# bayesiains/nflows

Hardware: NVIDIA H100
Metric: Flow.log_prob samples/sec, 10-layer RQ-NSF D=784 (higher is better)
Workload: dtype f32

## Files before the change

### nflows_b200/csrc/fused_spline.cuh

```cuda
#pragma once
#include "rq_spline.cuh"
#include "tc_common.cuh"

namespace nfk {
namespace tc {

constexpr int AFFINE_NB = 0;

constexpr int mog_nb(int mp) { return -mp / 8; }

template <int NB, bool TAILS>
struct FusedCfg {
    static constexpr bool AFFINE = NB == AFFINE_NB;
    static constexpr bool MOG = NB < 0;
    static constexpr int M = AFFINE ? 2 : (MOG ? -8 * NB : (TAILS ? 3 * NB - 1 : 3 * NB + 1));
    static constexpr int MP = AFFINE ? 2 : (M + 7) / 8 * 8;
    static constexpr int FPT = BN / (2 * MP);
    static constexpr int TF = 2 * FPT;
    static constexpr int TILE = TF * MP;
    static constexpr int LD = (TILE + 31) / 32 * 32;
    static_assert(FPT >= 1, "unsupported bin count for the fused kernels");
    static_assert(!(AFFINE && TAILS), "the affine epilogue has no tails");
    static_assert(!MOG || (!TAILS && MP <= 64), "mixture epilogue: no tails, at most 64 rows per feature");
};

struct MogOut {
    const float* u;
    const float* e;
    int64_t ldn;
    float eps;
    int C;
    int sample;
};

struct SplineOut {
    const float* bias;
    const float* x;
    float* y;
    __half* y_hi;
    __half* y_lo;
    const int32_t* t_cols;
    int t_col0;
    float out_scale;
    int64_t ldx, ldy, lds;
    int d_t;
    int inverse;
    float inv_acc_scale;
    SplineParams sp;
};

template <int NB, bool TAILS>
__device__ __forceinline__ int stg_chunk(int r, int c) {
    constexpr int C = FusedCfg<NB, TAILS>::FPT * FusedCfg<NB, TAILS>::MP / 4;
    return c ^ ((0x6530 >> (4 * (r & 3))) & 7) ^ ((C % 8 == 0 && c >= C) ? 4 : 0);
}

template <int NB, bool TAILS, int N, int LD = BN>
__device__ __forceinline__ void stage_sums(float* stg, const float (&sum)[N / 2], int wi, int lane) {
    static_assert(N <= LD && LD % 32 == 0, "staged row stride");
#pragma unroll
    for (int j = 0; j < N / 8; ++j)
#pragma unroll
        for (int h = 0; h < 2; ++h) {
            const int r = wi * 16 + (lane >> 2) + 8 * h, c = 2 * j + ((lane & 3) >> 1);
            *reinterpret_cast<float2*>(stg + r * LD + 4 * stg_chunk<NB, TAILS>(r, c) + 2 * (lane & 1)) =
                make_float2(sum[4 * j + 2 * h], sum[4 * j + 2 * h + 1]);
        }
}

template <int NB, bool TAILS>
struct SplineIn {
    float x[FusedCfg<NB, TAILS>::FPT];
    int col[FusedCfg<NB, TAILS>::FPT];
};
template <bool TAILS>
struct SplineIn<AFFINE_NB, TAILS> {};
template <int NB, bool TAILS>
__device__ __forceinline__ SplineIn<NB, TAILS> spline_inputs(const SplineOut& o, int n, int64_t row, bool row_ok, int fh) {
    constexpr int FPT = FusedCfg<NB, TAILS>::FPT, TF = FusedCfg<NB, TAILS>::TF;
    SplineIn<NB, TAILS> in;
    if constexpr (!FusedCfg<NB, TAILS>::AFFINE) {
        const int j0 = n * TF + fh * FPT;
#pragma unroll
        for (int f = 0; f < FPT; ++f) {
            const bool ok = row_ok && (j0 + f < o.d_t) && (!FusedCfg<NB, TAILS>::MOG || o.x != nullptr);
            in.col[f] = !ok ? 0 : (o.t_cols ? __ldg(o.t_cols + j0 + f) : o.t_col0 + j0 + f);
            in.x[f] = ok ? o.x[row * o.ldx + in.col[f]] : 0.0f;
        }
    }
    return in;
}

template <int NB, bool TAILS>
__device__ __forceinline__ void bias_tile_async(float* dst, const SplineOut& o, int n, int t) {
    constexpr int TILE = FusedCfg<NB, TAILS>::TILE, MP = FusedCfg<NB, TAILS>::MP;
    if constexpr (FusedCfg<NB, TAILS>::AFFINE) {
        if (t < TILE / 2) {
            const int e = n * TILE + 2 * t;
            const uint32_t bytes = e < o.d_t * MP ? 8u : 0u;
            asm volatile("cp.async.ca.shared.global [%0], [%1], 8, %2;" ::"r"(smem_u32(dst + 2 * t)), "l"(o.bias + (bytes ? e : 0)),
                         "r"(bytes)
                         : "memory");
        }
    } else if (t < TILE / 4) {
        const int e = n * TILE + 4 * t;
        const uint32_t bytes = e < o.d_t * MP ? 16u : 0u;
        asm volatile("cp.async.cg.shared.global [%0], [%1], 16, %2;" ::"r"(smem_u32(dst + 4 * t)), "l"(o.bias + (bytes ? e : 0)),
                     "r"(bytes)
                     : "memory");
    }
}
__device__ __forceinline__ void cp_async_wait_all() { asm volatile("cp.async.wait_all;" ::: "memory"); }

template <int NB, bool TAILS, int LD, bool BIAS_SMEM>
__device__ __forceinline__ void affine_tile(const SplineOut& o, const float* stg, int r, int n, int64_t row, bool row_ok, int fh,
                                            float& lad_row, const float* bias_tile) {
    using Cfg = FusedCfg<NB, TAILS>;
    constexpr int FPT = Cfg::FPT, TF = Cfg::TF, TILE = Cfg::TILE, C = FPT * 2 / 4;
    const int j0 = n * TF + fh * FPT;
    const int64_t c0 = (int64_t)o.t_col0 + j0;
    const float* b = o.bias + (int64_t)n * TILE + fh * FPT * 2;
    float lad = 0.0f;
    constexpr int G = 8;
#pragma unroll
    for (int g = 0; g < FPT; g += G) {
        float x[G];
#pragma unroll
        for (int f = 0; f < G; ++f) x[f] = (row_ok && j0 + g + f < o.d_t) ? __ldg(o.x + row * o.ldx + c0 + g + f) : 0.0f;
#pragma unroll
        for (int i = g / 2; i < (g + G) / 2; ++i) {
            const float4 s = *reinterpret_cast<const float4*>(stg + r * LD + 4 * stg_chunk<NB, TAILS>(r, fh * C + i));
            const float sv[4] = {s.x, s.y, s.z, s.w};
            float bv[4];
            if constexpr (BIAS_SMEM) {
                const float4 bq = *reinterpret_cast<const float4*>(bias_tile + fh * FPT * 2 + 4 * i);
                bv[0] = bq.x; bv[1] = bq.y; bv[2] = bq.z; bv[3] = bq.w;
            } else {
#pragma unroll
                for (int e = 0; e < 4; ++e) bv[e] = (j0 + 2 * i + e / 2 < o.d_t) ? __ldg(b + 4 * i + e) : 0.0f;
            }
#pragma unroll
            for (int h = 0; h < 2; ++h) {
                const int f = 2 * i + h;
                if (!(row_ok && j0 + f < o.d_t)) continue;
                const float u = fmaf(sv[2 * h], o.inv_acc_scale, bv[2 * h]);
                const float shift = fmaf(sv[2 * h + 1], o.inv_acc_scale, bv[2 * h + 1]);
                const float scale = __fadd_rn(softplus_torch(u, 1.0f, 1.0f), 1e-3f);
                const float xf = x[f - g];
                const float y = o.inverse ? __fdiv_rn(__fsub_rn(xf, shift), scale) : __fadd_rn(__fmul_rn(scale, xf), shift);
                o.y[row * o.ldy + c0 + f] = y;
                lad = __fadd_rn(lad, logf(scale));
            }
        }
    }
    lad_row += o.inverse ? -lad : lad;
}

template <int NB, bool TAILS, int LD>
__device__ __forceinline__ void mog_tile(const SplineOut& o, const MogOut& g, const float* stg, int r, int n, int64_t row, bool row_ok,
                                         int fh, const SplineIn<NB, TAILS>& in, float& lad_row, const float* bias_tile) {
    using Cfg = FusedCfg<NB, TAILS>;
    constexpr int MP = Cfg::MP, FPT = Cfg::FPT, TF = Cfg::TF, C4 = FPT * MP / 4, CMAX = MP / 3;
    constexpr float LOG_2PI = 1.8378770664093453f;
    const int j0 = n * TF + fh * FPT;
    float v[FPT * MP];
#pragma unroll
    for (int i = 0; i < C4; ++i) {
        const float4 s = *reinterpret_cast<const float4*>(stg + r * LD + 4 * stg_chunk<NB, TAILS>(r, fh * C4 + i));
        const float4 bq = *reinterpret_cast<const float4*>(bias_tile + fh * FPT * MP + 4 * i);
        v[4 * i + 0] = fmaf(s.x, o.inv_acc_scale, bq.x);
        v[4 * i + 1] = fmaf(s.y, o.inv_acc_scale, bq.y);
        v[4 * i + 2] = fmaf(s.z, o.inv_acc_scale, bq.z);
        v[4 * i + 3] = fmaf(s.w, o.inv_acc_scale, bq.w);
    }
    float lp = 0.0f;
#pragma unroll
    for (int f = 0; f < FPT; ++f) {
        if (!(row_ok && j0 + f < o.d_t)) continue;
        const float* q = v + f * MP;
        float lmax = -INFINITY;
#pragma unroll
        for (int c = 0; c < CMAX; ++c)
            if (c < g.C) lmax = fmaxf(lmax, q[3 * c]);
        float se = 0.0f;
#pragma unroll
        for (int c = 0; c < CMAX; ++c)
            if (c < g.C) se = __fadd_rn(se, expf(__fsub_rn(q[3 * c], lmax)));
        const int64_t col = (int64_t)o.t_col0 + j0 + f;
        if (!g.sample) {
            const float lse = logf(se), x = in.x[f];
            float t[CMAX];
            float tmax = -INFINITY;
#pragma unroll
            for (int c = 0; c < CMAX; ++c) {
                if (c >= g.C) continue;
                const float sigma = __fadd_rn(softplus_torch(q[3 * c + 2], 1.0f, 1.0f), g.eps);
                const float z = __fdiv_rn(__fsub_rn(x, q[3 * c + 1]), sigma);
                const float quad = __fadd_rn(__fadd_rn(LOG_2PI, __fmul_rn(2.0f, logf(sigma))), __fmul_rn(z, z));
                t[c] = __fsub_rn(__fsub_rn(__fsub_rn(q[3 * c], lmax), lse), __fmul_rn(0.5f, quad));
                tmax = fmaxf(tmax, t[c]);
            }
            float st = 0.0f;
#pragma unroll
            for (int c = 0; c < CMAX; ++c)
                if (c < g.C) st = __fadd_rn(st, expf(__fsub_rn(t[c], tmax)));
            lp = __fadd_rn(lp, __fadd_rn(logf(st), tmax));
        } else {
            const float uu = __ldg(g.u + row * g.ldn + j0 + f), ee = __ldg(g.e + row * g.ldn + j0 + f);
            float cum = 0.0f, mu = 0.0f, us = 0.0f;
            bool found = false;
#pragma unroll
            for (int c = 0; c < CMAX; ++c) {
                if (c >= g.C) continue;
                cum = __fadd_rn(cum, __fdiv_rn(expf(__fsub_rn(q[3 * c], lmax)), se));
                if (!found && (uu < cum || c == g.C - 1)) {
                    found = true;
                    mu = q[3 * c + 1];
                    us = q[3 * c + 2];
                }
            }
            const float sigma = __fadd_rn(softplus_torch(us, 1.0f, 1.0f), g.eps);
            o.y[row * o.ldy + col] = __fadd_rn(mu, __fmul_rn(ee, sigma));
        }
    }
    lad_row += lp;
}

template <int NB, bool TAILS, int LD = BN, bool BIAS_SMEM = false>
__device__ __forceinline__ void spline_tile(const SplineOut& o, const float* stg, int r, int n, int64_t row, bool row_ok, int fh,
                                            const SplineIn<NB, TAILS>& in, float& lad_row, int& flag,
                                            const float* bias_tile = nullptr) {
    using Cfg = FusedCfg<NB, TAILS>;
    if constexpr (Cfg::AFFINE) {
        affine_tile<NB, TAILS, LD, BIAS_SMEM>(o, stg, r, n, row, row_ok, fh, lad_row, bias_tile);
    } else {
        constexpr int MP = Cfg::MP, FPT = Cfg::FPT, TF = Cfg::TF, TILE = Cfg::TILE, C = FPT * MP / 4;
        const int j0 = n * TF + fh * FPT;
        float v[FPT * MP];
        const float* b = o.bias + (int64_t)n * TILE + fh * FPT * MP;
#pragma unroll
        for (int i = 0; i < C; ++i) {
            const float4 s = *reinterpret_cast<const float4*>(stg + r * LD + 4 * stg_chunk<NB, TAILS>(r, fh * C + i));
            const float sv[4] = {s.x, s.y, s.z, s.w};
            if constexpr (BIAS_SMEM) {
                const float4 bq = *reinterpret_cast<const float4*>(bias_tile + fh * FPT * MP + 4 * i);
                const float bv[4] = {bq.x, bq.y, bq.z, bq.w};
#pragma unroll
                for (int e = 0; e < 4; ++e) v[4 * i + e] = fmaf(sv[e], o.inv_acc_scale, bv[e]);
            } else {
#pragma unroll
                for (int e = 0; e < 4; ++e) {
                    const int c = 4 * i + e;
                    v[c] = fmaf(sv[e], o.inv_acc_scale, (j0 + c / MP < o.d_t) ? __ldg(b + c) : 0.0f);
                }
            }
        }
        float yy[FPT], ll[FPT];
        if (o.inverse) rqs_eval_lean<NB, TAILS, true, FPT, MP>(o.sp, in.x, v, yy, ll, flag);
        else rqs_eval_lean<NB, TAILS, false, FPT, MP>(o.sp, in.x, v, yy, ll, flag);
#pragma unroll
        for (int f = 0; f < FPT; ++f) {
            if (!(row_ok && j0 + f < o.d_t)) continue;
            lad_row += ll[f];
            if (o.y_hi) {
                __half hi, lo;
                split_f16(yy[f], o.out_scale, hi, lo, flag);
                o.y_hi[row * o.lds + in.col[f]] = hi;
                o.y_lo[row * o.lds + in.col[f]] = lo;
            } else {
                o.y[row * o.ldy + in.col[f]] = yy[f];
            }
        }
    }
}

}
}
```

### nflows_b200/csrc/nfk_coupling_step_tc.cu

```cuda
#include <stdlib.h>
#include <string.h>

#include <type_traits>

#include "fused_spline.cuh"

namespace nfk {
namespace tc {

constexpr int STEP_MAX_LAYERS = 9;
static_assert(STEP_MAX_LAYERS == NFK_STEP_MAX_LAYERS, "include/nfk.h: NfkStepRowTerms");
constexpr int STEP_MAX_HIDDEN = 256;
constexpr int STEP_DRAIN_TRUNK = 4;
constexpr int STEP_DRAIN_FINAL = 8;
constexpr int STEP_SLAB_BYTES = 2 * A_BYTES;
constexpr int STEP_R_BYTES = (STEP_MAX_HIDDEN / BK) * STEP_SLAB_BYTES;
constexpr int STEP_G0_STAGES = STEP_R_BYTES / STAGE_BYTES;
constexpr int STEP_S_OFF = STEP_R_BYTES;
constexpr int STEP_S_WG_BYTES = 32768;
constexpr int STEP_W_OFF = STEP_S_OFF + 2 * STEP_S_WG_BYTES;
constexpr int STEP_W_STAGES = 2;
constexpr int STEP_W_STAGE_BYTES = 2 * B_BYTES;
constexpr int STEP_BAR_OFF = STEP_W_OFF + STEP_W_STAGES * STEP_W_STAGE_BYTES;
constexpr int STEP_LAD_OFF = STEP_BAR_OFF + 256;
constexpr int STEP_BIAS_OFF = STEP_LAD_OFF + 512;
constexpr int STEP_SMEM_BYTES = STEP_BIAS_OFF + 2 * BN * 4 + 1024 ;
static_assert(64 * BN * 4 <= STEP_S_WG_BYTES && 4 * 2 * 64 * 64 <= STEP_S_WG_BYTES, "S");
static_assert(STEP_SMEM_BYTES <= 232448, "coupling-step kernel shared memory");
static_assert(STEP_MAX_HIDDEN / BK <= STEP_DRAIN_FINAL, "the final layer drains once (mma_final)");

template <int NB, bool TAILS>
struct StepFinal {
    static constexpr int TILE = FusedCfg<NB, TAILS>::TILE, LD = FusedCfg<NB, TAILS>::LD;
    static constexpr int STG_BYTES = 64 * LD * 4;
    static constexpr int RING_OFF = STEP_S_OFF + 2 * STG_BYTES;
    static constexpr int LO_OFF = TILE * ROW_BYTES;
    static constexpr int STAGE_BYTES = 2 * LO_OFF;
    static constexpr int STAGES = (STEP_BAR_OFF - RING_OFF) / STAGE_BYTES;
    static constexpr bool OWN_RING = STAGES > STEP_W_STAGES;
    static_assert(STG_BYTES <= STEP_S_WG_BYTES, "S");
    static_assert(RING_OFF % 512 == 0 && LO_OFF % 512 == 0 && STAGE_BYTES % 512 == 0, "final ring alignment");
    static_assert(!OWN_RING || (STAGES == 4 && RING_OFF >= STEP_S_OFF + STEP_S_WG_BYTES), "final ring");
    static_assert(112 + 2 * 8 * STAGES <= STEP_LAD_OFF - STEP_BAR_OFF, "its mbarriers follow bar_sfree");
};

#ifdef NFK_STEP_CLOCKS
constexpr int CLK_CTAS = 8, CLK_ROUNDS = 3, CLK_TILES = 128, CLK_TILE_STAMPS = 8;
constexpr int CLK_REC = 4 + CLK_TILES * CLK_TILE_STAMPS;
__device__ long long g_step_clocks[CLK_CTAS * CLK_ROUNDS * CLK_REC];
#define NFK_CLK(ptr, i) \
    do {                \
        if (ptr) (ptr)[i] = clock64(); \
    } while (0)
__device__ __forceinline__ long long* step_clock_record(int u, int t) {
    const int round = (u - (int)blockIdx.x) / (int)gridDim.x;
    if (t != 0 || blockIdx.x >= CLK_CTAS || round < 1 || round > CLK_ROUNDS) return nullptr;
    return g_step_clocks + ((int)blockIdx.x * CLK_ROUNDS + round - 1) * CLK_REC;
}
#define NFK_CLK_RECORD(u, t) step_clock_record(u, t)
#define NFK_CLK_TILE(rec, n) ((rec) && (n) < CLK_TILES ? (rec) + 4 + (n) * CLK_TILE_STAMPS : nullptr)
#else
#define NFK_CLK(ptr, i) \
    do {                \
    } while (0)
#define NFK_CLK_RECORD(u, t) ((long long*)nullptr)
#define NFK_CLK_TILE(rec, n) ((long long*)nullptr)
#endif

constexpr int SL_RELU_OUT = 1;
constexpr int SL_ADD_SKIP = 2;
constexpr int SL_SAVE_SKIP = 4;
constexpr int SL_SPLIT_RELU = 8;
constexpr int SL_ACT_SHIFT = 8;
constexpr int SL_ACT_MASK = 15;

__host__ __device__ __forceinline__ int layer_act(int lf) {
    const int a = (lf >> SL_ACT_SHIFT) & SL_ACT_MASK;
    return a ? a : NFK_ACT_RELU;
}

template <int ACT>
__device__ __forceinline__ void act_frag(float (&v)[64]) {
#pragma unroll
    for (int i = 0; i < 64; ++i) v[i] = nfk_act(ACT, v[i]);
}

__device__ __forceinline__ void act_fragment(int act, float (&v)[64]) {
    switch (act) {
        case NFK_ACT_RELU: act_frag<NFK_ACT_RELU>(v); break;
        case NFK_ACT_TANH: act_frag<NFK_ACT_TANH>(v); break;
        case NFK_ACT_ELU: act_frag<NFK_ACT_ELU>(v); break;
        case NFK_ACT_LEAKY_RELU: act_frag<NFK_ACT_LEAKY_RELU>(v); break;
        case NFK_ACT_GELU: act_frag<NFK_ACT_GELU>(v); break;
        case NFK_ACT_SILU: act_frag<NFK_ACT_SILU>(v); break;
    }
}

struct StepParams {
    const float* bias_trunk;
    float* skip_buf;
    int H, K0, num_layers;
    int layer_flags[STEP_MAX_LAYERS];
    float acc_scale[STEP_MAX_LAYERS], inv_acc_scale[STEP_MAX_LAYERS];
    float act_scale;
    __half* h_hi;
    __half* h_lo;
    int64_t ldh;
    SplineOut o;
    float* lad_accum;
    int32_t* flags;
    int64_t n_rows;
    int num_m_tiles, num_n_tiles;
};

struct StepTermParams : StepParams {
    const float* add[STEP_MAX_LAYERS];
    int64_t ld_add[STEP_MAX_LAYERS];
};

struct StepMogParams : StepTermParams {
    MogOut mog;
};

template <int NB, bool TERMS>
using StepParamsOf = typename std::conditional<FusedCfg<NB, false>::MOG, StepMogParams,
                                               typename std::conditional<TERMS, StepTermParams, StepParams>::type>::type;

__device__ __forceinline__ void put_pair(uint8_t* base, int slab_stride, int lo_off, int r, int col, float x0, float x1, float scale,
                                         float& amax) {
    x0 *= scale; x1 *= scale;
    amax = fmaxf(amax, fmaxf(fabsf(x0), fabsf(x1)));
    const __half2 h = __floats2half2_rn(x0, x1);
    const float2 hf = __half22float2(h);
    const __half2 l = __floats2half2_rn(x0 - hf.x, x1 - hf.y);
    const int k = col & 31;
    uint8_t* q = base + (col >> 5) * slab_stride + r * 64 + (((k >> 3) ^ ((r >> 1) & 3)) << 4) + (k & 7) * 2;
    *reinterpret_cast<__half2*>(q) = h;
    *reinterpret_cast<__half2*>(q + lo_off) = l;
}

__device__ __forceinline__ void consumers_sync() { asm volatile("bar.sync 3, 256;" ::: "memory"); }
constexpr int STEP_BAR_TURN = 4;
constexpr int STEP_BAR_LAD = 6;

template <int N, int MH>
__device__ __forceinline__ void mma_final(float (&acc)[MH][N / 2], Ring& r, int num_k, uint32_t a_res, int lane, int turn,
                                          uint32_t lo_off, [[maybe_unused]] long long* clk) {
    int prev = -1;
    for (int j = 0; j < num_k; ++j) {
        mbar_wait(r.full + 8 * r.stage, r.phase);
        if (j == 0) NFK_CLK(clk, 1);
        if (j == num_k - 1) NFK_CLK(clk, 2);
        if (turn >= 0 && j == num_k - 1) {
            __threadfence_block();
            pair_arrive(turn);
        }
        const uint32_t sw = r.base + r.stage * r.stage_bytes;
        const uint64_t w_hi = make_smem_desc(sw), w_lo = make_smem_desc(sw + lo_off);
        wgmma_fence();
#pragma unroll
        for (int m = 0; m < MH; ++m) {
            const uint32_t sa = a_res + (uint32_t)j * STEP_SLAB_BYTES + m * (A_BYTES / 2);
            const uint64_t a_hi = make_smem_desc(sa), a_lo = make_smem_desc(sa + A_BYTES);
#pragma unroll
            for (int kk = 0; kk < BK / 16; ++kk) {
                const uint64_t adv = (uint64_t)(kk * 2);
                wgmma_f16<N>(acc[m], a_lo + adv, w_hi + adv, (j | kk) != 0);
                wgmma_f16<N>(acc[m], a_hi + adv, w_lo + adv, 1);
            }
#pragma unroll
            for (int kk = 0; kk < BK / 16; ++kk) {
                const uint64_t adv = (uint64_t)(kk * 2);
                wgmma_f16<N>(acc[m], a_hi + adv, w_hi + adv, 1);
            }
        }
        wgmma_commit();
        if (prev >= 0) {
            wgmma_wait<1>();
            __syncwarp();
            if (lane == 0) mbar_arrive(r.empty + 8 * prev, MH);
        }
        prev = r.stage;
        r.advance();
    }
    wgmma_wait<0>();
    NFK_CLK(clk, 3);
    __syncwarp();
    if (lane == 0) mbar_arrive(r.empty + 8 * prev, MH);
}

template <int NB, bool TAILS, bool TERMS, bool ACT>
__global__ void __launch_bounds__(THREADS, 1)
rq_coupling_step_kernel(const __grid_constant__ CUtensorMap map_a_hi, const __grid_constant__ CUtensorMap map_a_lo,
                        const __grid_constant__ CUtensorMap map_w0_hi, const __grid_constant__ CUtensorMap map_w0_lo,
                        const __grid_constant__ CUtensorMap map_wt_hi, const __grid_constant__ CUtensorMap map_wt_lo,
                        const __grid_constant__ CUtensorMap map_wf_hi, const __grid_constant__ CUtensorMap map_wf_lo,
                        const StepParamsOf<NB, TERMS> p) {
    using F = StepFinal<NB, TAILS>;
    constexpr int TILE = F::TILE;
    extern __shared__ uint8_t smem_raw[];
    const uint32_t smem_base = (smem_u32(smem_raw) + 1023u) & ~1023u;
    uint8_t* smem_gen = smem_raw + (smem_base - smem_u32(smem_raw));
    const uint32_t bars = smem_base + STEP_BAR_OFF;
    Ring ring0{smem_base, bars, bars + 8 * STEP_G0_STAGES, STEP_G0_STAGES, (uint32_t)STAGE_BYTES};
    Ring ring1{smem_base + STEP_W_OFF, bars + 64, bars + 64 + 8 * STEP_W_STAGES, STEP_W_STAGES, (uint32_t)STEP_W_STAGE_BYTES};
    Ring ring_own{smem_base + F::RING_OFF, bars + 112, bars + 112 + 8 * F::STAGES, F::STAGES, (uint32_t)F::STAGE_BYTES};
    Ring& ringf = F::OWN_RING ? ring_own : ring1;
    constexpr uint32_t lo_f = F::OWN_RING ? F::LO_OFF : B_BYTES;
    const uint32_t bar_rfree = bars + 96;
    const uint32_t bar_sfree = bars + 104;
    const int warp = threadIdx.x >> 5, lane = threadIdx.x & 31;
    const int H = p.H;
    const int num_k0 = (p.K0 + BK - 1) / BK, num_kh = H / BK;
    const int nch = (H + BN - 1) / BN;
    const bool trunk_only = p.h_hi != nullptr;

    if (threadIdx.x == 0) {
        for (int s = 0; s < STEP_G0_STAGES; ++s) { mbar_init(ring0.full + 8 * s, 1); mbar_init(ring0.empty + 8 * s, 8); }
        for (int s = 0; s < STEP_W_STAGES; ++s) { mbar_init(ring1.full + 8 * s, 1); mbar_init(ring1.empty + 8 * s, 8); }
        mbar_init(bar_rfree, 8);
        if constexpr (F::OWN_RING) {
            for (int s = 0; s < F::STAGES; ++s) { mbar_init(ring_own.full + 8 * s, 1); mbar_init(ring_own.empty + 8 * s, 8); }
            mbar_init(bar_sfree, 1);
        }
        asm volatile("fence.mbarrier_init.release.cluster;" ::: "memory");
        prefetch_tmap(&map_a_hi); prefetch_tmap(&map_a_lo); prefetch_tmap(&map_w0_hi); prefetch_tmap(&map_w0_lo);
        prefetch_tmap(&map_wt_hi); prefetch_tmap(&map_wt_lo); prefetch_tmap(&map_wf_hi); prefetch_tmap(&map_wf_lo);
    }
    __syncthreads();

    if (warp < 4) {
        asm volatile("setmaxnreg.dec.sync.aligned.u32 40;" ::: "memory");
        if (warp == 0 && elect_one()) {
            uint32_t rphase = 0, sphase = 0;
            for (int u = blockIdx.x; u < p.num_m_tiles; u += gridDim.x) {
                if (u != (int)blockIdx.x) { mbar_wait(bar_rfree, rphase); rphase ^= 1; }
                for (int c = 0; c < nch; ++c)
                    for (int ks = 0; ks < num_k0; ++ks) produce_slab(ring0, &map_a_hi, &map_a_lo, &map_w0_hi, &map_w0_lo, ks, u * BM, c * BN);
                for (int l = 1; l < p.num_layers; ++l)
                    for (int c = 0; c < nch; ++c)
                        for (int ks = 0; ks < num_kh; ++ks) produce_w_slab(ring1, &map_wt_hi, &map_wt_lo, ks, (l - 1) * H + c * BN);
                if (trunk_only) continue;
                if (F::OWN_RING && p.num_n_tiles > 1) {
                    mbar_wait(bar_sfree, sphase);
                    sphase ^= 1;
                    Ring w = ring1;
                    for (int s = 0; s < STEP_W_STAGES; ++s) {
                        mbar_wait(w.empty + 8 * w.stage, w.phase ^ 1);
                        w.advance();
                    }
                    for (int n = 0; n < p.num_n_tiles; ++n)
                        for (int ks = 0; ks < num_kh; ++ks) produce_w_slab(ring_own, &map_wf_hi, &map_wf_lo, ks, n * TILE, TILE, F::LO_OFF);
                } else {
                    for (int n = 0; n < p.num_n_tiles; ++n)
                        for (int ks = 0; ks < num_kh; ++ks) produce_w_slab(ring1, &map_wf_hi, &map_wf_lo, ks, n * TILE, TILE);
                }
            }
        }
        return;
    }
    asm volatile("setmaxnreg.inc.sync.aligned.u32 232;" ::: "memory");
    const int wg = (warp >> 2) - 1, wi = warp & 3, q = lane & 3;
    const int t = threadIdx.x - 128 * (1 + wg);
    const int r_loc = t >> 1, fh = t & 1;
    uint8_t* R = smem_gen;
    uint8_t* S = smem_gen + STEP_S_OFF + wg * STEP_S_WG_BYTES;
    float* stg = reinterpret_cast<float*>(S);
    float* const bias_wg = reinterpret_cast<float*>(smem_gen + STEP_BIAS_OFF) + wg * BN;
    float* skip = p.skip_buf + (size_t)blockIdx.x * BM * H;
    int flag = 0;
    for (int u = blockIdx.x; u < p.num_m_tiles; u += gridDim.x) {
        const int64_t m0 = (int64_t)u * BM;
        int rt[2];
        rt[0] = wg * 64 + wi * 16 + (lane >> 2);
        rt[1] = rt[0] + 8;
        [[maybe_unused]] long long* const clk = NFK_CLK_RECORD(u, t);
        NFK_CLK(clk, 2 * wg);
        for (int l = 0; l < p.num_layers; ++l) {
            const int lf = p.layer_flags[l];
            [[maybe_unused]] const int act = layer_act(lf);
            const bool to_global = trunk_only && l == p.num_layers - 1;
            const float as = p.acc_scale[l], ias = p.inv_acc_scale[l];
            float amax = 0.0f;
            for (int c = 0; c < nch; ++c) {
                const int cb = c * BN + 2 * q;
                float sum[64];
#pragma unroll
                for (int j = 0; j < 16; ++j) {
                    const int col = cb + 8 * j;
                    [[maybe_unused]] float2 tv[2] = {make_float2(0.0f, 0.0f), make_float2(0.0f, 0.0f)};
                    if constexpr (TERMS) {
                        const float* ta = p.add[l];
                        if (ta != nullptr && col < H) {
#pragma unroll
                            for (int h = 0; h < 2; ++h) {
                                const int64_t row = m0 + rt[h];
                                if (row < p.n_rows) tv[h] = __ldg(reinterpret_cast<const float2*>(ta + row * p.ld_add[l] + col));
                            }
                        }
                    }
#pragma unroll
                    for (int e = 0; e < 2; ++e) {
                        const float b = col < H ? __ldg(p.bias_trunk + l * H + col + e) * as : 0.0f;
#pragma unroll
                        for (int h = 0; h < 2; ++h) {
                            float sk = ((lf & SL_ADD_SKIP) && col < H) ? skip[rt[h] * H + col + e] : 0.0f;
                            if constexpr (TERMS) sk += e ? tv[h].y : tv[h].x;
                            sum[4 * j + 2 * h + e] = fmaf(sk, as, b);
                        }
                    }
                }
                if (l == 0) mma_tile(sum, ring0, num_k0, STEP_DRAIN_TRUNK, wg, lane);
                else mma_tile(sum, ring1, num_kh, STEP_DRAIN_TRUNK, wg, lane, smem_base);
#pragma unroll
                for (int i = 0; i < 64; ++i) {
                    float x = sum[i] * ias;
                    if (!ACT && (lf & SL_RELU_OUT)) x = fmaxf(x, 0.0f);
                    sum[i] = x;
                }
                if (ACT && (lf & SL_RELU_OUT)) act_fragment(act, sum);
                if (lf & SL_SAVE_SKIP) {
#pragma unroll
                    for (int j = 0; j < 16; ++j)
#pragma unroll
                        for (int h = 0; h < 2; ++h)
                            if (cb + 8 * j < H)
                                *reinterpret_cast<float2*>(skip + rt[h] * H + cb + 8 * j) = make_float2(sum[4 * j + 2 * h], sum[4 * j + 2 * h + 1]);
                }
                if (lf & SL_SPLIT_RELU) {
                    if constexpr (ACT) {
                        act_fragment(act, sum);
                    } else {
#pragma unroll
                        for (int i = 0; i < 64; ++i) sum[i] = fmaxf(sum[i], 0.0f);
                    }
                }
                if (to_global) {
#pragma unroll
                    for (int h = 0; h < 2; ++h) {
                        const int64_t row = m0 + rt[h];
                        if (row >= p.n_rows) continue;
                        float am = 0.0f;
#pragma unroll
                        for (int j = 0; j < 16; ++j) {
                            const int col = cb + 8 * j;
                            if (col >= H) continue;
                            const float x0 = sum[4 * j + 2 * h] * p.act_scale, x1 = sum[4 * j + 2 * h + 1] * p.act_scale;
                            am = fmaxf(am, fmaxf(fabsf(x0), fabsf(x1)));
                            const __half2 hh = __floats2half2_rn(x0, x1);
                            const float2 hf = __half22float2(hh);
                            *reinterpret_cast<__half2*>(p.h_hi + row * p.ldh + col) = hh;
                            *reinterpret_cast<__half2*>(p.h_lo + row * p.ldh + col) = __floats2half2_rn(x0 - hf.x, x1 - hf.y);
                        }
                        if (!(am <= 65000.0f)) flag |= 4;
                    }
                    continue;
                }
                const bool into_r = c == nch - 1;
                if (into_r) {
                    if (l == 0) consumers_sync();
                } else {
                    wg_sync(wg);
                }
#pragma unroll
                for (int h = 0; h < 2; ++h) {
                    float am = 0.0f;
#pragma unroll
                    for (int j = 0; j < 16; ++j) {
                        const int cc = 8 * j + 2 * q;
                        if (c * BN + cc >= H) continue;
                        if (into_r)
                            put_pair(R, STEP_SLAB_BYTES, A_BYTES, rt[h], c * BN + cc, sum[4 * j + 2 * h], sum[4 * j + 2 * h + 1], p.act_scale, am);
                        else
                            put_pair(S, 2 * A_BYTES / 2, A_BYTES / 2, rt[h] - wg * 64, cc, sum[4 * j + 2 * h], sum[4 * j + 2 * h + 1],
                                     p.act_scale, am);
                    }
                    if (m0 + rt[h] < p.n_rows) amax = fmaxf(amax, am);
                }
                if (into_r && nch > 1) {
                    wg_sync(wg);
                    for (int i = t; i < 4 * 2 * 256; i += 128) {
                        const int part = i >> 8, k = i & 255;
                        const uint4 v = reinterpret_cast<const uint4*>(S + part * 4096)[k];
                        reinterpret_cast<uint4*>(R + (part >> 1) * STEP_SLAB_BYTES + (part & 1) * A_BYTES + wg * 4096)[k] = v;
                    }
                }
            }
            if (!(amax <= 65000.0f)) flag |= 4;
            if (!to_global) {
                asm volatile("fence.proxy.async.shared::cta;" ::: "memory");
                wg_sync(wg);
            }
        }
        NFK_CLK(clk, 2 * wg + 1);
        if (trunk_only) {
            __syncwarp();
            if (lane == 0) mbar_arrive(bar_rfree);
            continue;
        }
        if (p.num_n_tiles == 1) {
            const int64_t srow = m0 + wg * 64 + r_loc;
            const bool row_ok = srow < p.n_rows;
            const SplineIn<NB, TAILS> in = spline_inputs<NB, TAILS>(p.o, 0, srow, row_ok, fh);
            bias_tile_async<NB, TAILS>(bias_wg, p.o, 0, t);
            float acc[1][TILE / 2] = {};
            mma_final<TILE, 1>(acc, ring1, num_kh, smem_base + wg * (A_BYTES / 2), lane, -1, B_BYTES, nullptr);
            __syncwarp();
            if (lane == 0) mbar_arrive(bar_rfree);
            stage_sums<NB, TAILS, TILE, F::LD>(stg, acc[0], wi, lane);
            cp_async_wait_all();
            wg_sync(wg);
            float lad_row = 0.0f;
            if constexpr (FusedCfg<NB, TAILS>::MOG)
                mog_tile<NB, TAILS, F::LD>(p.o, p.mog, stg, r_loc, 0, srow, row_ok, fh, in, lad_row, bias_wg);
            else
                spline_tile<NB, TAILS, F::LD, true>(p.o, stg, r_loc, 0, srow, row_ok, fh, in, lad_row, flag, bias_wg);
            const float other = __shfl_xor_sync(0xffffffffu, lad_row, 1);
            if (p.lad_accum && fh == 0 && row_ok) p.lad_accum[srow] += lad_row + other;
            continue;
        }
        consumers_sync();
        if constexpr (F::OWN_RING)
            if (t == 0 && wg == 0) mbar_arrive(bar_sfree);
        float* const stg_pp = reinterpret_cast<float*>(smem_gen + STEP_S_OFF + wg * F::STG_BYTES);
        const int nt = p.num_n_tiles;
        int64_t srow[2];
        bool row_ok[2];
        float lad[2] = {0.0f, 0.0f};
#pragma unroll
        for (int m = 0; m < 2; ++m) {
            srow[m] = m0 + 64 * m + r_loc;
            row_ok[m] = srow[m] < p.n_rows;
        }
        for (int n = 0; n < nt; ++n) {
            if ((n & 1) != wg) {
                for (int ks = 0; ks < num_kh; ++ks) ringf.advance();
                continue;
            }
            [[maybe_unused]] long long* const clk_t = NFK_CLK_TILE(clk, n);
            SplineIn<NB, TAILS> in[2];
#pragma unroll
            for (int m = 0; m < 2; ++m) in[m] = spline_inputs<NB, TAILS>(p.o, n, srow[m], row_ok[m], fh);
            NFK_CLK(clk_t, 0);
            if (n > 0) pair_wait(STEP_BAR_TURN + wg);
            bias_tile_async<NB, TAILS>(bias_wg, p.o, n, t);
            float acc[2][TILE / 2] = {};
            mma_final<TILE, 2>(acc, ringf, num_kh, smem_base, lane, n + 1 < nt ? STEP_BAR_TURN + (wg ^ 1) : -1, lo_f, clk_t);
            if (n + 2 >= nt) {
                __syncwarp();
                if (lane == 0) mbar_arrive(bar_rfree);
            }
#pragma unroll
            for (int m = 0; m < 2; ++m) {
                wg_sync(wg);
                stage_sums<NB, TAILS, TILE, F::LD>(stg_pp, acc[m], wi, lane);
                if (m == 0) cp_async_wait_all();
                wg_sync(wg);
                NFK_CLK(clk_t, 4 + 2 * m);
                if constexpr (FusedCfg<NB, TAILS>::MOG)
                    mog_tile<NB, TAILS, F::LD>(p.o, p.mog, stg_pp, r_loc, n, srow[m], row_ok[m], fh, in[m], lad[m], bias_wg);
                else
                    spline_tile<NB, TAILS, F::LD, true>(p.o, stg_pp, r_loc, n, srow[m], row_ok[m], fh, in[m], lad[m], flag, bias_wg);
                NFK_CLK(clk_t, 5 + 2 * m);
            }
        }
        float* lad_x = reinterpret_cast<float*>(smem_gen + STEP_LAD_OFF);
#pragma unroll
        for (int m = 0; m < 2; ++m) lad[m] += __shfl_xor_sync(0xffffffffu, lad[m], 1);
        if (wg == 1) {
            if (fh == 0) {
                lad_x[r_loc] = lad[0];
                lad_x[64 + r_loc] = lad[1];
            }
            __threadfence_block();
            pair_arrive(STEP_BAR_LAD);
        } else {
            pair_wait(STEP_BAR_LAD);
            if (p.lad_accum && fh == 0)
#pragma unroll
                for (int m = 0; m < 2; ++m)
                    if (row_ok[m]) p.lad_accum[srow[m]] += lad[m] + lad_x[64 * m + r_loc];
        }
    }
    if (flag && p.flags) atomicOr(p.flags, flag);
}

template <int NB, bool TAILS, bool TERMS, bool ACT>
static int start_step(const CUtensorMap (&m)[8], int grid, StepParamsOf<NB, TERMS>& p, cudaStream_t st) {
    static DeviceOnce attr_once;
    int attr_dev = 0;
    if (attr_once.pending(&attr_dev)) {
        cudaError_t e = cudaFuncSetAttribute(rq_coupling_step_kernel<NB, TAILS, TERMS, ACT>, cudaFuncAttributeMaxDynamicSharedMemorySize,
                                             STEP_SMEM_BYTES);
        if (e != cudaSuccess) return fail(NFK_E_CUDA, "cudaFuncSetAttribute(smem=%d): %s", STEP_SMEM_BYTES, cudaGetErrorString(e));
        attr_once.mark(attr_dev);
    }
    rq_coupling_step_kernel<NB, TAILS, TERMS, ACT><<<grid, THREADS, STEP_SMEM_BYTES, st>>>(m[0], m[1], m[2], m[3], m[4], m[5], m[6],
                                                                                         m[7], p);
    return check_launch("rq_coupling_step_kernel");
}

template <int NB, bool TAILS, bool TERMS>
static int launch_step(const NfkCouplingStep* d, StepParamsOf<NB, TERMS>& p, cudaStream_t st) {
    using Cfg = FusedCfg<NB, TAILS>;
    const int H = p.H, L = p.num_layers - 1;
    CUtensorMap ma_hi, ma_lo, mw0_hi, mw0_lo, mwt_hi, mwt_lo, mwf_hi, mwf_lo;
    int rc;
    if ((rc = make_map(&ma_hi, (const __half*)d->a_hi, p.n_rows, p.K0, d->lda, BM))) return rc;
    if ((rc = make_map(&ma_lo, (const __half*)d->a_lo, p.n_rows, p.K0, d->lda, BM))) return rc;
    if ((rc = make_map(&mw0_hi, (const __half*)d->w0_hi, H, p.K0, d->ldw0, BN))) return rc;
    if ((rc = make_map(&mw0_lo, (const __half*)d->w0_lo, H, p.K0, d->ldw0, BN))) return rc;
    mwt_hi = mw0_hi; mwt_lo = mw0_lo;
    if (L > 0) {
        if ((rc = make_map(&mwt_hi, (const __half*)d->wt_hi, (int64_t)L * H, H, d->ldwt, BN))) return rc;
        if ((rc = make_map(&mwt_lo, (const __half*)d->wt_lo, (int64_t)L * H, H, d->ldwt, BN))) return rc;
    }
    mwf_hi = mw0_hi; mwf_lo = mw0_lo;
    p.num_n_tiles = 0;
    if (!p.h_hi) {
        const int packed_rows = p.o.d_t * Cfg::MP;
        if ((rc = make_map(&mwf_hi, (const __half*)d->wp_hi, packed_rows, H, d->ldwp, Cfg::TILE))) return rc;
        if ((rc = make_map(&mwf_lo, (const __half*)d->wp_lo, packed_rows, H, d->ldwp, Cfg::TILE))) return rc;
        p.num_n_tiles = (p.o.d_t + Cfg::TF - 1) / Cfg::TF;
    }
    const int grid = p.num_m_tiles < sm_count() ? p.num_m_tiles : sm_count();
    NFK_REQUIRE(d->workspace_bytes >= (size_t)grid * (size_t)H * BM * 4, "workspace too small: %zu bytes given, %zu needed",
                d->workspace_bytes, (size_t)grid * (size_t)H * BM * 4);
    bool act = false;
    for (int l = 0; l < p.num_layers; ++l) act = act || ((p.layer_flags[l] >> SL_ACT_SHIFT) & SL_ACT_MASK) != 0;
    const CUtensorMap maps[8] = {ma_hi, ma_lo, mw0_hi, mw0_lo, mwt_hi, mwt_lo, mwf_hi, mwf_lo};
    return act ? start_step<NB, TAILS, TERMS, true>(maps, grid, p, st) : start_step<NB, TAILS, TERMS, false>(maps, grid, p, st);
}

}
}

using namespace nfk;

extern "C" int nfk_rq_coupling_step_supported(int32_t num_bins, int32_t linear_tails, int32_t hidden_features, int32_t in_features,
                                              int32_t num_square_layers) {
    const bool bins_ok = (num_bins == 8 || num_bins == 10 || num_bins == 4 || num_bins == 16);
    return (bins_ok && hidden_features >= 32 && hidden_features <= tc::STEP_MAX_HIDDEN && hidden_features % 32 == 0 && in_features >= 8 &&
            in_features % 8 == 0 && num_square_layers >= 0 && num_square_layers < tc::STEP_MAX_LAYERS) ? 1 : 0;
}

extern "C" size_t nfk_rq_coupling_step_workspace_bytes(int32_t hidden_features) {
    return (size_t)tc::sm_count() * (size_t)hidden_features * tc::BM * 4;
}

static int check_row_terms(const NfkCouplingStep* d, const NfkStepRowTerms* terms, bool* has_terms) {
    *has_terms = false;
    if (!terms) return NFK_OK;
    for (int l = 0; l < tc::STEP_MAX_LAYERS; ++l) {
        const NfkRowTerm& t = terms->layer[l];
        if (!t.add) continue;
        NFK_REQUIRE(l <= d->num_square_layers, "row term on layer %d, but the trunk has %d layers", l, 1 + d->num_square_layers);
        NFK_REQUIRE(t.ld >= d->hidden_features, "row term of layer %d: ld=%lld is less than the hidden width %d", l, (long long)t.ld,
                    d->hidden_features);
        NFK_REQUIRE(t.ld % 2 == 0 && (reinterpret_cast<uintptr_t>(t.add) & 7) == 0,
                    "row term of layer %d must be 8-byte aligned with an even ld (it is read as float2)", l);
        *has_terms = true;
    }
    NFK_REQUIRE(!*has_terms || d->h_hi == nullptr, "row terms are not supported with the trunk-only output (h_hi)");
    return NFK_OK;
}

static int check_trunk(const NfkCouplingStep* d) {
    NFK_REQUIRE(d->a_hi && d->a_lo && d->w0_hi && d->w0_lo && d->bias_trunk && d->layer_flags && d->workspace, "NULL pointer");
    NFK_REQUIRE(d->num_square_layers == 0 || (d->wt_hi && d->wt_lo && d->wt_exps), "square-layer weights missing");
    NFK_REQUIRE(d->lda % 8 == 0 && d->ldw0 % 8 == 0 && (d->num_square_layers == 0 || d->ldwt % 8 == 0), "row pitches must be multiples of 8");
    NFK_REQUIRE(aligned16(d->a_hi) && aligned16(d->a_lo) && aligned16(d->w0_hi) && aligned16(d->w0_lo) && aligned16(d->bias_trunk) &&
                    aligned16(d->workspace) && (d->num_square_layers == 0 || (aligned16(d->wt_hi) && aligned16(d->wt_lo))),
                "operands must be 16-byte aligned");
    NFK_REQUIRE(d->n_rows < (1ll << 31), "n_rows too large for one launch");
    for (int l = 0; l <= d->num_square_layers; ++l) {
        const int lf = d->layer_flags[l];
        const int e = l == 0 ? d->a_exp + d->w0_exp : d->act_exp + d->wt_exps[l - 1];
        NFK_REQUIRE(!((lf & tc::SL_ADD_SKIP) && (lf & tc::SL_RELU_OUT)), "layer %d: skip add after a relu output is not supported", l);
        NFK_REQUIRE(act_valid(tc::layer_act(lf)), "layer %d: unknown activation code %d in the layer flags", l,
                    (lf >> tc::SL_ACT_SHIFT) & tc::SL_ACT_MASK);
        NFK_REQUIRE(e >= -60 && e <= 60, "scale exponent out of range");
    }
    return NFK_OK;
}

static void trunk_params(const NfkCouplingStep* d, const NfkStepRowTerms* terms, bool has_terms, tc::StepTermParams& p) {
    const int L = d->num_square_layers;
    memset(&p, 0, sizeof(p));
    p.bias_trunk = d->bias_trunk; p.skip_buf = (float*)d->workspace; p.H = d->hidden_features; p.K0 = d->in_features;
    p.num_layers = 1 + L; p.act_scale = ldexpf(1.0f, d->act_exp);
    for (int l = 0; l <= L; ++l) {
        const int e = l == 0 ? d->a_exp + d->w0_exp : d->act_exp + d->wt_exps[l - 1];
        p.layer_flags[l] = d->layer_flags[l];
        p.acc_scale[l] = ldexpf(1.0f, e);
        p.inv_acc_scale[l] = ldexpf(1.0f, -e);
    }
    p.flags = d->flags; p.n_rows = d->n_rows;
    p.num_m_tiles = (int)((d->n_rows + tc::BM - 1) / tc::BM);
    if (has_terms)
        for (int l = 0; l <= L; ++l) {
            p.add[l] = terms->layer[l].add;
            p.ld_add[l] = terms->layer[l].ld;
        }
}

static void final_params(const NfkCouplingStep* d, tc::StepTermParams& p) {
    p.o.bias = d->bias_packed; p.o.x = d->x; p.o.y = d->y; p.o.y_hi = (__half*)d->y_hi; p.o.y_lo = (__half*)d->y_lo;
    p.o.t_cols = d->t_cols; p.o.t_col0 = d->t_col0; p.o.out_scale = ldexpf(1.0f, d->y_exp); p.o.ldx = d->ldx; p.o.ldy = d->ldy;
    p.o.lds = d->lds; p.o.d_t = d->d_t; p.o.inverse = d->inverse; p.o.inv_acc_scale = ldexpf(1.0f, -(d->act_exp + d->wp_exp));
    p.lad_accum = d->lad_accum;
}

static int coupling_step(const NfkCouplingStep* d, const NfkStepRowTerms* terms, void* stream) {
    NFK_REQUIRE(d, "NULL descriptor");
    NFK_REQUIRE(d->n_rows >= 0 && d->hidden_features >= 1 && d->in_features >= 1, "bad sizes");
    bool has_terms = false;
    int rc = check_row_terms(d, terms, &has_terms);
    if (rc) return rc;
    if (d->n_rows == 0) return NFK_OK;
    const bool trunk_only = d->h_hi != nullptr;
    const int nb = trunk_only && !d->spline ? 8 : (d->spline ? d->spline->num_bins : 0);
    const int lt = trunk_only && !d->spline ? 1 : (d->spline ? d->spline->linear_tails : 0);
    NFK_REQUIRE(trunk_only || d->spline, "spline descriptor missing");
    NFK_REQUIRE(nfk_rq_coupling_step_supported(nb, lt, d->hidden_features, d->in_features, d->num_square_layers),
                "coupling-step kernel does not take num_bins=%d hidden=%d in_features=%d square layers=%d", nb, d->hidden_features,
                d->in_features, d->num_square_layers);
    if ((rc = check_trunk(d))) return rc;
    if (trunk_only) {
        NFK_REQUIRE(d->h_lo && d->ldh % 8 == 0 && aligned16(d->h_hi) && aligned16(d->h_lo), "bad trunk output pair");
    } else {
        NFK_REQUIRE(d->wp_hi && d->wp_lo && d->bias_packed && d->x && d->d_t >= 1, "NULL pointer");
        NFK_REQUIRE((d->y != nullptr) != (d->y_hi != nullptr), "give either y (fp32 outputs) or y_hi / y_lo (their fp16 split pair)");
        NFK_REQUIRE((d->y_hi == nullptr) == (d->y_lo == nullptr) && d->y_exp >= -60 && d->y_exp <= 60, "bad pair output");
        NFK_REQUIRE(d->t_cols || d->t_col0 >= 0, "t_cols is NULL and t_col0 is negative");
// ... 133 lines not shown
```

Before: 2.045 million.

## Keep final-layer accumulators in registers via quad shuffles instead of smem staging

For spline epilogues with a 96-wide tile, the final GEMM accumulators are redistributed within each quad using xor shuffles, so each thread holds whole spline units. The shared-memory staging round trip and its two workgroup barriers per row-half are skipped. The freed staging space is handed to the final-layer ring, giving it 8 stages instead of 4. This changes the thread-to-row mapping for the epilogue and the log-det reduction, and adds shuffle work and register pressure.

```diff
diff --git a/nflows_b200/csrc/fused_spline.cuh b/nflows_b200/csrc/fused_spline.cuh
--- a/nflows_b200/csrc/fused_spline.cuh
+++ b/nflows_b200/csrc/fused_spline.cuh
@@ -68,6 +68,70 @@
         }
 }
 
+constexpr __host__ __device__ int quad_pair_a(int k, int i) { return k == 0 ? i : 4 * (i >> 1) + (i & 1); }
+constexpr __host__ __device__ int quad_pair_b(int J, int k, int i) { return quad_pair_a(k, i) + (k == 0 ? 4 * J : 2); }
+constexpr __host__ __device__ int quad_slot(int J, int c) {
+    return 4 * (c >> 3) + 2 * ((c >> 2) & 1) + (c & 1) + 4 * J * ((c >> 1) & 1);
+}
+
+template <int N>
+__device__ __forceinline__ void quad_units(float (&x)[N / 2], int lane) {
+    constexpr int J = N / 16;
+#pragma unroll
+    for (int k = 0; k < 2; ++k) {
+        const bool hi = (lane >> k) & 1;
+#pragma unroll
+        for (int i = 0; i < 4 * J; ++i) {
+            const int a = quad_pair_a(k, i), b = quad_pair_b(J, k, i);
+            const float recv = __shfl_xor_sync(0xffffffffu, hi ? x[a] : x[b], 1 << k);
+            x[a] = hi ? recv : x[a];
+            x[b] = hi ? x[b] : recv;
+        }
+    }
+}
+
+template <int NB, bool TAILS, int LD, bool BIAS_SMEM>
+__device__ __forceinline__ void gather_staged(float (&v)[FusedCfg<NB, TAILS>::FPT * FusedCfg<NB, TAILS>::MP], const SplineOut& o,
+                                              const float* stg, int r, int n, int fh, const float* bias_tile) {
+    using Cfg = FusedCfg<NB, TAILS>;
+    constexpr int MP = Cfg::MP, FPT = Cfg::FPT, TF = Cfg::TF, TILE = Cfg::TILE, C = FPT * MP / 4;
+    const int j0 = n * TF + fh * FPT;
+    const float* b = o.bias + (int64_t)n * TILE + fh * FPT * MP;
+#pragma unroll
+    for (int i = 0; i < C; ++i) {
+        const float4 s = *reinterpret_cast<const float4*>(stg + r * LD + 4 * stg_chunk<NB, TAILS>(r, fh * C + i));
+        const float sv[4] = {s.x, s.y, s.z, s.w};
+        if constexpr (BIAS_SMEM) {
+            const float4 bq = *reinterpret_cast<const float4*>(bias_tile + fh * FPT * MP + 4 * i);
+            const float bv[4] = {bq.x, bq.y, bq.z, bq.w};
+#pragma unroll
+            for (int e = 0; e < 4; ++e) v[4 * i + e] = fmaf(sv[e], o.inv_acc_scale, bv[e]);
+        } else {
+#pragma unroll
+            for (int e = 0; e < 4; ++e) {
+                const int c = 4 * i + e;
+                v[c] = fmaf(sv[e], o.inv_acc_scale, (j0 + c / MP < o.d_t) ? __ldg(b + c) : 0.0f);
+            }
+        }
+    }
+}
+
+template <int NB, bool TAILS>
+__device__ __forceinline__ void gather_regs(float (&v)[FusedCfg<NB, TAILS>::FPT * FusedCfg<NB, TAILS>::MP], const SplineOut& o,
+                                            float (&sum)[FusedCfg<NB, TAILS>::TILE / 2], int lane, const float* bias_tile) {
+    constexpr int U = FusedCfg<NB, TAILS>::FPT * FusedCfg<NB, TAILS>::MP, J = FusedCfg<NB, TAILS>::TILE / 16;
+    static_assert(2 * U == FusedCfg<NB, TAILS>::TILE && U % 8 == 0, "a quad holds 4 whole units");
+    quad_units<FusedCfg<NB, TAILS>::TILE>(sum, lane);
+    const float* bt = bias_tile + (lane & 1) * U;
+#pragma unroll
+    for (int i = 0; i < U / 4; ++i) {
+        const float4 bq = *reinterpret_cast<const float4*>(bt + 4 * i);
+        const float bv[4] = {bq.x, bq.y, bq.z, bq.w};
+#pragma unroll
+        for (int e = 0; e < 4; ++e) v[4 * i + e] = fmaf(sum[quad_slot(J, 4 * i + e)], o.inv_acc_scale, bv[e]);
+    }
+}
+
 template <int NB, bool TAILS>
 struct SplineIn {
     float x[FusedCfg<NB, TAILS>::FPT];
@@ -226,6 +290,30 @@
     lad_row += lp;
 }
 
+template <int NB, bool TAILS>
+__device__ __forceinline__ void spline_eval(const SplineOut& o, float (&v)[FusedCfg<NB, TAILS>::FPT * FusedCfg<NB, TAILS>::MP],
+                                            int n, int64_t row, bool row_ok, int fh, const SplineIn<NB, TAILS>& in, float& lad_row,
+                                            int& flag) {
+    constexpr int MP = FusedCfg<NB, TAILS>::MP, FPT = FusedCfg<NB, TAILS>::FPT;
+    const int j0 = n * FusedCfg<NB, TAILS>::TF + fh * FPT;
+    float yy[FPT], ll[FPT];
+    if (o.inverse) rqs_eval_lean<NB, TAILS, true, FPT, MP>(o.sp, in.x, v, yy, ll, flag);
+    else rqs_eval_lean<NB, TAILS, false, FPT, MP>(o.sp, in.x, v, yy, ll, flag);
+#pragma unroll
+    for (int f = 0; f < FPT; ++f) {
+        if (!(row_ok && j0 + f < o.d_t)) continue;
+        lad_row += ll[f];
+        if (o.y_hi) {
+            __half hi, lo;
+            split_f16(yy[f], o.out_scale, hi, lo, flag);
+            o.y_hi[row * o.lds + in.col[f]] = hi;
+            o.y_lo[row * o.lds + in.col[f]] = lo;
+        } else {
+            o.y[row * o.ldy + in.col[f]] = yy[f];
+        }
+    }
+}
+
 template <int NB, bool TAILS, int LD = BN, bool BIAS_SMEM = false>
 __device__ __forceinline__ void spline_tile(const SplineOut& o, const float* stg, int r, int n, int64_t row, bool row_ok, int fh,
                                             const SplineIn<NB, TAILS>& in, float& lad_row, int& flag,
@@ -234,45 +322,11 @@
     if constexpr (Cfg::AFFINE) {
         affine_tile<NB, TAILS, LD, BIAS_SMEM>(o, stg, r, n, row, row_ok, fh, lad_row, bias_tile);
     } else {
-        constexpr int MP = Cfg::MP, FPT = Cfg::FPT, TF = Cfg::TF, TILE = Cfg::TILE, C = FPT * MP / 4;
-        const int j0 = n * TF + fh * FPT;
-        float v[FPT * MP];
-        const float* b = o.bias + (int64_t)n * TILE + fh * FPT * MP;
-#pragma unroll
-        for (int i = 0; i < C; ++i) {
-            const float4 s = *reinterpret_cast<const float4*>(stg + r * LD + 4 * stg_chunk<NB, TAILS>(r, fh * C + i));
-            const float sv[4] = {s.x, s.y, s.z, s.w};
-            if constexpr (BIAS_SMEM) {
-                const float4 bq = *reinterpret_cast<const float4*>(bias_tile + fh * FPT * MP + 4 * i);
-                const float bv[4] = {bq.x, bq.y, bq.z, bq.w};
-#pragma unroll
-                for (int e = 0; e < 4; ++e) v[4 * i + e] = fmaf(sv[e], o.inv_acc_scale, bv[e]);
-            } else {
-#pragma unroll
-                for (int e = 0; e < 4; ++e) {
-                    const int c = 4 * i + e;
-                    v[c] = fmaf(sv[e], o.inv_acc_scale, (j0 + c / MP < o.d_t) ? __ldg(b + c) : 0.0f);
-                }
-            }
-        }
-        float yy[FPT], ll[FPT];
-        if (o.inverse) rqs_eval_lean<NB, TAILS, true, FPT, MP>(o.sp, in.x, v, yy, ll, flag);
-        else rqs_eval_lean<NB, TAILS, false, FPT, MP>(o.sp, in.x, v, yy, ll, flag);
-#pragma unroll
-        for (int f = 0; f < FPT; ++f) {
-            if (!(row_ok && j0 + f < o.d_t)) continue;
-            lad_row += ll[f];
-            if (o.y_hi) {
-                __half hi, lo;
-                split_f16(yy[f], o.out_scale, hi, lo, flag);
-                o.y_hi[row * o.lds + in.col[f]] = hi;
-                o.y_lo[row * o.lds + in.col[f]] = lo;
-            } else {
-                o.y[row * o.ldy + in.col[f]] = yy[f];
-            }
-        }
-    }
-}
-
-}
-}
+        float v[Cfg::FPT * Cfg::MP];
+        gather_staged<NB, TAILS, LD, BIAS_SMEM>(v, o, stg, r, n, fh, bias_tile);
+        spline_eval<NB, TAILS>(o, v, n, row, row_ok, fh, in, lad_row, flag);
+    }
+}
+
+}
+}
diff --git a/nflows_b200/csrc/nfk_coupling_step_tc.cu b/nflows_b200/csrc/nfk_coupling_step_tc.cu
--- a/nflows_b200/csrc/nfk_coupling_step_tc.cu
+++ b/nflows_b200/csrc/nfk_coupling_step_tc.cu
@@ -32,15 +32,16 @@
 template <int NB, bool TAILS>
 struct StepFinal {
     static constexpr int TILE = FusedCfg<NB, TAILS>::TILE, LD = FusedCfg<NB, TAILS>::LD;
+    static constexpr bool REGS = !FusedCfg<NB, TAILS>::AFFINE && !FusedCfg<NB, TAILS>::MOG && TILE == 96;
     static constexpr int STG_BYTES = 64 * LD * 4;
-    static constexpr int RING_OFF = STEP_S_OFF + 2 * STG_BYTES;
+    static constexpr int RING_OFF = REGS ? STEP_S_OFF : STEP_S_OFF + 2 * STG_BYTES;
     static constexpr int LO_OFF = TILE * ROW_BYTES;
     static constexpr int STAGE_BYTES = 2 * LO_OFF;
     static constexpr int STAGES = (STEP_BAR_OFF - RING_OFF) / STAGE_BYTES;
     static constexpr bool OWN_RING = STAGES > STEP_W_STAGES;
     static_assert(STG_BYTES <= STEP_S_WG_BYTES, "S");
     static_assert(RING_OFF % 512 == 0 && LO_OFF % 512 == 0 && STAGE_BYTES % 512 == 0, "final ring alignment");
-    static_assert(!OWN_RING || (STAGES == 4 && RING_OFF >= STEP_S_OFF + STEP_S_WG_BYTES), "final ring");
+    static_assert(REGS ? STAGES == 8 : (!OWN_RING || (STAGES == 4 && RING_OFF >= STEP_S_OFF + STEP_S_WG_BYTES)), "final ring");
     static_assert(112 + 2 * 8 * STAGES <= STEP_LAD_OFF - STEP_BAR_OFF, "its mbarriers follow bar_sfree");
 };
 
@@ -263,6 +264,7 @@
     const int wg = (warp >> 2) - 1, wi = warp & 3, q = lane & 3;
     const int t = threadIdx.x - 128 * (1 + wg);
     const int r_loc = t >> 1, fh = t & 1;
+    const int pp_row = F::REGS ? wi * 16 + (lane >> 2) + 8 * (q >> 1) : r_loc, pp_fh = F::REGS ? q & 1 : fh;
     uint8_t* R = smem_gen;
     uint8_t* S = smem_gen + STEP_S_OFF + wg * STEP_S_WG_BYTES;
     float* stg = reinterpret_cast<float*>(S);
@@ -429,7 +431,7 @@
         float lad[2] = {0.0f, 0.0f};
 #pragma unroll
         for (int m = 0; m < 2; ++m) {
-            srow[m] = m0 + 64 * m + r_loc;
+            srow[m] = m0 + 64 * m + pp_row;
             row_ok[m] = srow[m] < p.n_rows;
         }
         for (int n = 0; n < nt; ++n) {
@@ -440,7 +442,7 @@
             [[maybe_unused]] long long* const clk_t = NFK_CLK_TILE(clk, n);
             SplineIn<NB, TAILS> in[2];
 #pragma unroll
-            for (int m = 0; m < 2; ++m) in[m] = spline_inputs<NB, TAILS>(p.o, n, srow[m], row_ok[m], fh);
+            for (int m = 0; m < 2; ++m) in[m] = spline_inputs<NB, TAILS>(p.o, n, srow[m], row_ok[m], pp_fh);
             NFK_CLK(clk_t, 0);
             if (n > 0) pair_wait(STEP_BAR_TURN + wg);
             bias_tile_async<NB, TAILS>(bias_wg, p.o, n, t);
@@ -450,36 +452,53 @@
                 __syncwarp();
                 if (lane == 0) mbar_arrive(bar_rfree);
             }
-#pragma unroll
-            for (int m = 0; m < 2; ++m) {
+            if constexpr (F::REGS) {
+#pragma unroll
+                for (int m = 0; m < 2; ++m)
+#pragma unroll
+                    for (int i = 0; i < TILE / 2; ++i) asm volatile("" : "+f"(acc[m][i])::"memory");
+                cp_async_wait_all();
                 wg_sync(wg);
-                stage_sums<NB, TAILS, TILE, F::LD>(stg_pp, acc[m], wi, lane);
-                if (m == 0) cp_async_wait_all();
-                wg_sync(wg);
-                NFK_CLK(clk_t, 4 + 2 * m);
-                if constexpr (FusedCfg<NB, TAILS>::MOG)
-                    mog_tile<NB, TAILS, F::LD>(p.o, p.mog, stg_pp, r_loc, n, srow[m], row_ok[m], fh, in[m], lad[m], bias_wg);
-                else
-                    spline_tile<NB, TAILS, F::LD, true>(p.o, stg_pp, r_loc, n, srow[m], row_ok[m], fh, in[m], lad[m], flag, bias_wg);
-                NFK_CLK(clk_t, 5 + 2 * m);
+#pragma unroll
+                for (int m = 0; m < 2; ++m) {
+                    float v[FusedCfg<NB, TAILS>::FPT * FusedCfg<NB, TAILS>::MP];
+                    gather_regs<NB, TAILS>(v, p.o, acc[m], lane, bias_wg);
+                    NFK_CLK(clk_t, 4 + 2 * m);
+                    spline_eval<NB, TAILS>(p.o, v, n, srow[m], row_ok[m], pp_fh, in[m], lad[m], flag);
+                    NFK_CLK(clk_t, 5 + 2 * m);
+                }
+            } else {
+#pragma unroll
+                for (int m = 0; m < 2; ++m) {
+                    wg_sync(wg);
+                    stage_sums<NB, TAILS, TILE, F::LD>(stg_pp, acc[m], wi, lane);
+                    if (m == 0) cp_async_wait_all();
+                    wg_sync(wg);
+                    NFK_CLK(clk_t, 4 + 2 * m);
+                    if constexpr (FusedCfg<NB, TAILS>::MOG)
+                        mog_tile<NB, TAILS, F::LD>(p.o, p.mog, stg_pp, r_loc, n, srow[m], row_ok[m], fh, in[m], lad[m], bias_wg);
+                    else
+                        spline_tile<NB, TAILS, F::LD, true>(p.o, stg_pp, r_loc, n, srow[m], row_ok[m], fh, in[m], lad[m], flag, bias_wg);
+                    NFK_CLK(clk_t, 5 + 2 * m);
+                }
             }
         }
         float* lad_x = reinterpret_cast<float*>(smem_gen + STEP_LAD_OFF);
 #pragma unroll
         for (int m = 0; m < 2; ++m) lad[m] += __shfl_xor_sync(0xffffffffu, lad[m], 1);
         if (wg == 1) {
-            if (fh == 0) {
-                lad_x[r_loc] = lad[0];
-                lad_x[64 + r_loc] = lad[1];
+            if (pp_fh == 0) {
+                lad_x[pp_row] = lad[0];
+                lad_x[64 + pp_row] = lad[1];
             }
             __threadfence_block();
             pair_arrive(STEP_BAR_LAD);
         } else {
             pair_wait(STEP_BAR_LAD);
-            if (p.lad_accum && fh == 0)
+            if (p.lad_accum && pp_fh == 0)
 #pragma unroll
                 for (int m = 0; m < 2; ++m)
-                    if (row_ok[m]) p.lad_accum[srow[m]] += lad[m] + lad_x[64 * m + r_loc];
+                    if (row_ok[m]) p.lad_accum[srow[m]] += lad[m] + lad_x[64 * m + pp_row];
         }
     }
     if (flag && p.flags) atomicOr(p.flags, flag);
```

Result: faster. 2.076 million, median of 6 (+1.5%).
